# christian-rauch/MultiMotionFusion

Hardware: AMD Instinct MI355X
Metric: frames/sec @ 640x480 (dense ICP+RGB tracking + surfel fusion); Gauss-Newton iteration kernel (ICP + RGB JtJ-reduce) achieved HBM GB/s vs peak (higher is better)
Workload: dtype f32

## Files before the change

### include/mmf_hip.h

```cpp
#ifndef MMF_HIP_H_
#define MMF_HIP_H_

#include <stddef.h>
#include <stdint.h>

#ifdef __cplusplus
extern "C" {
#endif

#define MMF_ABI_VERSION 3

typedef enum {
    MMF_OK = 0,
    MMF_ERR_INVALID = -1,
    MMF_ERR_HIP = -2,
    MMF_ERR_NO_DEVICE = -3,
    MMF_ERR_STATE = -4
} mmf_status;

typedef struct mmf_ctx mmf_ctx;
typedef struct mmf_odom mmf_odom;

typedef struct {
    int16_t zero_x, zero_y;
// ... 248 lines not shown
int mmf_fusion_set_frame_to_frame_rgb(mmf_fusion *f, int val);
int mmf_fusion_set_depth_cutoff(mmf_fusion *f, float val);
int mmf_fusion_set_confidence_threshold(mmf_fusion *f, float val);
int mmf_fusion_set_enable_multiple_models(mmf_fusion *f, int val);
int mmf_fusion_get_config(mmf_fusion *f, mmf_fusion_config *out);
int mmf_fusion_set_shard(mmf_fusion *f, int rank, int world);
int mmf_fusion_owns_model(mmf_fusion *f, int index);
int mmf_fusion_set_model_pose(mmf_fusion *f, int index, const float pose[16]);
typedef struct mmf_shard mmf_shard;
int mmf_shard_unique_id(char id[128]);
int mmf_shard_create(mmf_ctx *ctx, int rank, int world, const char id[128], mmf_shard **out);
int mmf_shard_attach(mmf_ctx *ctx, int rank, int world, void *nccl_comm, mmf_shard **out);
void mmf_shard_destroy(mmf_shard *s);
int mmf_shard_broadcast_frame(mmf_shard *s, uint8_t *rgb, float *depth, uint8_t *mask, int width, int height, int root);
int mmf_shard_post_frame(mmf_shard *s, uint8_t *rgb, float *depth, uint8_t *mask, int width, int height, int root, int slot);
int mmf_shard_wait_frame(mmf_shard *s, int slot);
int mmf_shard_gather_poses(mmf_shard *s, mmf_fusion *f);
int mmf_shard_gather_poses_begin(mmf_shard *s, mmf_fusion *f);
int mmf_shard_gather_poses_end(mmf_shard *s, mmf_fusion *f);
int mmf_shard_gather_maps(mmf_shard *s, mmf_fusion *f, const int *labels, int spixel_size, float *out_dev);
int mmf_fusion_last_timings(mmf_fusion *f, double *tracking_s, double *frame_s);
int mmf_fusion_set_segmentation_callback(mmf_fusion *f, mmf_segmentation_fn fn, void *user);
int mmf_fusion_export_poses(mmf_fusion *f, const char *export_dir);
int mmf_fusion_pose_log(mmf_fusion *f, int index, long long *ts, float *p7, int max_entries, int *n_out);
int mmf_debug_expf(mmf_ctx *ctx, const float *x_dev, int n, float *out_mmf_dev, float *out_packed_dev);
int mmf_debug_set_gn_fused(int on);
int mmf_gn_chain_status(int *recoveries, int *one_launch_chain_in_use);
int mmf_debug_force_gn_fault(int n);
int mmf_debug_set_sparse_check(int on);
int mmf_debug_set_sparse_groups(int n);
int mmf_debug_odom_sparse_outside(mmf_odom *o, unsigned *outside, int *walked_by_extent, int rect[9]);
int mmf_debug_set_mid_predict(int on);
int mmf_debug_set_splat_bound(int mode);
int mmf_debug_set_pass_batch(int mode);
int mmf_debug_set_prep_rect(int on);
int mmf_debug_set_xcd(int on);
unsigned mmf_debug_xcd_block(unsigned block, unsigned blocks);
int mmf_debug_set_begin_rider(int on);
int mmf_debug_begin_rider_count(void);
int mmf_debug_set_track_cull(int mode);
int mmf_debug_depth_keys(mmf_ctx *ctx, const float *z_dev, int n, float max_depth, unsigned *fast_dev, unsigned *divided_dev);
int mmf_compute_fusion_weight(const float pose[16], const float last_pose[16], float multiplier, float *out);

int mmf_match_descriptors(mmf_ctx *ctx, const float *query, int nq, const float *train, int nt, int dim,
                          float max_distance, int *train_idx, float *distance);

typedef struct mmf_superpoint mmf_superpoint;
int mmf_superpoint_create(mmf_ctx *ctx, const float *const *weights, int max_width, int max_height,
                          int max_keypoints, mmf_superpoint **out);
void mmf_superpoint_destroy(mmf_superpoint *sp);
int mmf_superpoint_forward(mmf_superpoint *sp, const uint8_t *image, int width, int height, int channels);
int mmf_superpoint_download(mmf_superpoint *sp, int which, float *host, size_t count);
int mmf_superpoint_get_features(mmf_superpoint *sp, const uint8_t *image, int width, int height, int channels,
                                float conf_thresh, int nms_dist, int border, int *xy, float *conf, float *desc,
                                int *count);
int mmf_superpoint_conv(mmf_ctx *ctx, const float *in, int height, int width, int cin, const float *w,
                        const float *bias, int cout, int taps, int relu, int pool, int nt, float *out);

int mmf_slic_downsample(mmf_ctx *ctx, const int *labels, int width, int height, int spixel_size, const float *image,
                        int channels, int channel, int thresholded, float min_threshold, float *out, int *counts_out);
int mmf_slic_downsample_rgb(mmf_ctx *ctx, const int *labels, int width, int height, int spixel_size, const uint8_t *rgb,
                            int channels, uint8_t *out);
int mmf_slic_upsample_u8(mmf_ctx *ctx, const int *labels, int width, int height, const uint8_t *map, int nspix,
                         uint8_t *out);

typedef struct {
// ... 46 lines not shown
```

### multimotionfusion_amd/_capi.py

```python
import ctypes as C
import os

_PKG_DIR = os.path.dirname(os.path.abspath(__file__))
LIB_PATH = os.environ.get("MMF_HIP_LIB") or os.path.join(_PKG_DIR, "libmmf_hip.so")

MMF_NUM_PYRS = 3


class MmfError(RuntimeError):
    def __init__(self, status, message):
        super().__init__(f"mmf status {status}: {message}")
        self.status = status


class mmf_camera(C.Structure):
    _fields_ = [("fx", C.c_float), ("fy", C.c_float), ("cx", C.c_float), ("cy", C.c_float)]


class mmf_dataterm(C.Structure):
    _fields_ = [("zero_x", C.c_int16), ("zero_y", C.c_int16), ("one_x", C.c_int16), ("one_y", C.c_int16),
                ("diff", C.c_float), ("valid", C.c_uint8), ("pad_", C.c_uint8 * 3)]


class mmf_odom_stats(C.Structure):
# ... 176 lines not shown
                             _vp, C.POINTER(mmf_segmentation_model), _ip, _ip]),
    "mmf_crf_last": (_i, [_vp, C.POINTER(mmf_crf_info), C.POINTER(mmf_segmentation_model), _i, _vp, _vp, _vp, _vp]),
    "mmf_fusion_export_poses": (_i, [_vp, C.c_char_p]),
    "mmf_fusion_pose_log": (_i, [_vp, _i, C.POINTER(C.c_longlong), _fp, _i, _ip]),
    "mmf_compute_fusion_weight": (_i, [_fp, _fp, _f, _fp]),
    "mmf_fusion_preallocate_models": (_i, [_vp, C.c_uint]),
    "mmf_shard_unique_id": (_i, [C.c_char_p]),
    "mmf_shard_create": (_i, [_vp, _i, _i, C.c_char_p, C.POINTER(_vp)]),
    "mmf_shard_attach": (_i, [_vp, _i, _i, _vp, C.POINTER(_vp)]),
    "mmf_shard_destroy": (None, [_vp]),
    "mmf_shard_broadcast_frame": (_i, [_vp, _vp, _vp, _vp, _i, _i, _i]),
    "mmf_shard_post_frame": (_i, [_vp, _vp, _vp, _vp, _i, _i, _i, _i]),
    "mmf_shard_wait_frame": (_i, [_vp, _i]),
    "mmf_shard_gather_poses": (_i, [_vp, _vp]),
    "mmf_shard_gather_poses_begin": (_i, [_vp, _vp]),
    "mmf_shard_gather_poses_end": (_i, [_vp, _vp]),
    "mmf_shard_gather_maps": (_i, [_vp, _vp, _vp, _i, _vp]),
    "mmf_debug_expf": (_i, [_vp, _vp, _i, _vp, _vp]),
    "mmf_model_surfel_arrays": (_i, [_vp, C.POINTER(_vp), C.POINTER(_vp), C.POINTER(_vp), C.POINTER(C.c_uint)]),
    "mmf_debug_set_gn_fused": (_i, [_i]),
    "mmf_debug_set_mid_predict": (_i, [_i]),
    "mmf_debug_force_gn_fault": (_i, [_i]),
    "mmf_debug_set_sparse_check": (_i, [_i]),
    "mmf_debug_set_pass_batch": (_i, [_i]),
    "mmf_debug_set_prep_rect": (_i, [_i]),
    "mmf_debug_set_xcd": (_i, [_i]),
    "mmf_debug_xcd_block": (C.c_uint, [C.c_uint, C.c_uint]),
    "mmf_debug_set_begin_rider": (_i, [_i]),
    "mmf_debug_begin_rider_count": (_i, []),
    "mmf_debug_set_sparse_groups": (_i, [_i]),
    "mmf_debug_odom_sparse_outside": (_i, [_vp, C.POINTER(C.c_uint), C.POINTER(_i), C.POINTER(_i)]),
    "mmf_gn_chain_status": (_i, [C.POINTER(_i), C.POINTER(_i)]),
    "mmf_debug_set_splat_bound": (_i, [_i]),
    "mmf_debug_set_track_cull": (_i, [_i]),
    "mmf_debug_depth_keys": (_i, [_vp, _vp, _i, _f, _vp, _vp]),
    "mmf_fusion_set_shard": (_i, [_vp, _i, _i]),
    "mmf_fusion_owns_model": (_i, [_vp, _i]),
    "mmf_fusion_set_model_pose": (_i, [_vp, _i, _fp]),
    "mmf_fusion_last_timings": (_i, [_vp, C.POINTER(C.c_double), C.POINTER(C.c_double)]),
    "mmf_odom_enable_timing": (_i, [_vp, _i]),
    "mmf_odom_get_timing": (_i, [_vp, C.POINTER(mmf_odom_timing)]),
    "mmf_model_set_max_depth": (_i, [_vp, _f]),
    "mmf_model_set_confidence_threshold": (_i, [_vp, _f]),
    "mmf_model_confidence_threshold": (_f, [_vp]),
    "mmf_model_id": (_i, [_vp]),
}

_lib = None


def load():
    global _lib
    if _lib is not None:
        return _lib
    if not os.path.exists(LIB_PATH):
        raise ImportError(
            f"{LIB_PATH} is missing: build it with `python -m multimotionfusion_amd.build` "
            "(hipcc, gfx950). multimotionfusion_amd has no CPU fallback.")
    import torch
    lib = C.CDLL(LIB_PATH)
    for name, (restype, argtypes) in SIGNATURES.items():
        if os.environ.get("MMF_HIP_LIB") and name.startswith("mmf_debug_") and not hasattr(lib, name):
            continue
        fn = getattr(lib, name)
        fn.restype = restype
        fn.argtypes = argtypes
# ... 12 lines not shown
```

### multimotionfusion_amd/csrc/mmf_hip.hip

```cpp
#include "../../include/mmf_hip.h"

#include <hip/hip_runtime.h>
#include <hip/hip_ext.h>

#include <algorithm>
#include <array>
#include <atomic>
#include <cfloat>
#include <chrono>
#include <cmath>
#include <cstddef>
#include <cstdio>
#include <cstdlib>
#include <condition_variable>
#include <cstring>
#include <map>
#include <mutex>
#include <thread>
#include <new>
#include <string>
#include <tuple>
#include <type_traits>
#include <utility>
#include <vector>
// ... 2468 lines not shown
extern "C" int mmf_model_predict_indices(mmf_model* m, int time, float depth_cutoff, int time_delta) {
    return model_predict_indices(m, time, depth_cutoff, time_delta, false);
}

static unsigned* model_thumb_counts(mmf_model* m) { return &m->totals[4]; }
static dim3 splat_grid(size_t bound, bool deep = false) {
    const unsigned wgs = tunables().splat_wgs > 0 ? (unsigned)tunables().splat_wgs : (deep ? 2048u : 512u);
    const size_t one_per_thread = (bound + 255) / 256;
    return dim3((unsigned)std::max<size_t>(1, std::min<size_t>(one_per_thread, wgs)));
}
#ifdef MMF_SPLAT_COUNT
extern "C" int mmf_debug_splat_counts(unsigned long long out[4], int reset) {
    MMF_HIP_TRY(hipDeviceSynchronize());
    MMF_HIP_TRY(hipMemcpyFromSymbol(out, HIP_SYMBOL(g_splat_dbg), 32));
    if (reset) {
        const unsigned long long z[4] = {0, 0, 0, 0};
        MMF_HIP_TRY(hipMemcpyToSymbol(HIP_SYMBOL(g_splat_dbg), z, 32));
    }
    return MMF_OK;
}
#endif
extern "C" int mmf_debug_depth_keys(mmf_ctx* c, const float* z_dev, int n, float max_depth, unsigned* fast_dev, unsigned* divided_dev) {
    MMF_REQUIRE(c && z_dev && fast_dev && divided_dev && n > 0, "mmf_debug_depth_keys: bad argument");
    MMF_HIP_TRY(hipSetDevice(c->device));
    hipLaunchKernelGGL(depth_key_probe_kernel, grid1d((size_t)n), dim3(256), 0, c->stream, z_dev, n, max_depth, fast_dev, divided_dev);
    MMF_HIP_TRY(hipGetLastError());
    return MMF_OK;
}
static std::atomic<int> g_splat_bound{-2};
extern "C" int mmf_debug_set_splat_bound(int mode) {
    g_splat_bound.store(mode < 0 ? -1 : (mode ? 1 : 0));
    return MMF_OK;
}
static int model_combined_predict(mmf_model* m, float depth_cutoff, int time, int max_time, int time_delta,
                                  const uint8_t* fill_rgb, const float* fill_depth, int frame_to_frame_rgb, int lost) {
    MMF_REQUIRE(m != nullptr, "mmf_model_combined_predict: null model");
    mmf_ctx* c = m->ctx;
    MMF_HIP_TRY(hipSetDevice(c->device));
    ++m->tex_gen;
    ++m->thumb_gen;
    m->spl_nz_known = false;
    SplatArgs a;
    inverse4f_host(m->pose, a.t_inv.m);
    a.t_inv_dev = m->t_inv_dev;
    a.abort_dev = m->abort_dev;
    a.c = make_cam(m, false);
    a.cols = m->width, a.rows = m->height;
    a.maxDepth = depth_cutoff;
    a.confThreshold = m->conf_threshold;
    a.time = time, a.maxTime = max_time, a.timeDelta = time_delta;
    const unsigned launch_count = m->count_pending ? m->count_bound : m->count;
    const int bound_mode = g_splat_bound.load() == -2 ? tunables().splat_bound : g_splat_bound.load();
    const size_t npix_s = (size_t)m->width * m->height;
    const bool deep_store = (size_t)launch_count >= 2 * npix_s;
    const bool deep = bound_mode < 0 ? deep_store : bound_mode != 0;
    a.early_z = deep ? 1 : 0;
    a.rays = m->rays;
    const bool keep_box = m->boxes != nullptr && !(fill_rgb && fill_depth) && !deep && m->id != 0;
    if (keep_box) {
        ++m->kgen, ++m->sgen;
        const size_t plausible = std::min<size_t>(launch_count, (size_t)m->count * 2 + 8192);
        if (launch_count)
            hipLaunchKernelGGL(splat_box_kernel, splat_grid(plausible, plausible >= npix_s / 2), dim3(256), 0, c->stream, m->set[m->cur],
                               (int)launch_count, a, m->keys, m->count_pending ? m->totals : nullptr, m->boxes, m->kgen);
        hipLaunchKernelGGL(splat_resolve_keep_box_kernel, dim3(splat_tile_grid(m->width, m->height)), dim3(256), 0, c->stream, m->set[m->cur], a, m->keys,
                           m->image, m->vertexConf, m->normalRadius, m->time_tex, model_thumb_counts(m), (int)(m->thumb_gen & 1), m->boxes, m->kgen,
                           m->sgen);
        m->spl_nz_known = true;
        MMF_HIP_TRY(hipGetLastError());
        return MMF_OK;
    }
    if (launch_count)
        hipLaunchKernelGGL(deep ? splat_kernel<true> : splat_kernel<false>, splat_grid(launch_count, (size_t)launch_count >= npix_s / 2), dim3(256), 0, c->stream,
                           m->set[m->cur], (int)launch_count, a, m->keys, m->count_pending ? m->totals : nullptr);
    if (fill_rgb && fill_depth) {
        hipLaunchKernelGGL(splat_resolve_fill_kernel, dim3(splat_tile_grid(m->width, m->height)), dim3(256), 0,
                           c->stream, m->set[m->cur], a, m->keys, m->image, m->vertexConf, m->normalRadius, m->time_tex, fill_depth,
                           fill_rgb, lost ? 1 : 0, (lost || frame_to_frame_rgb) ? 1 : 0, m->fill_vertex, m->fill_normal,
                           m->fill_image, model_thumb_counts(m), (int)(m->thumb_gen & 1));
    } else
        hipLaunchKernelGGL(splat_resolve_kernel, dim3(splat_tile_grid(m->width, m->height)), dim3(256), 0, c->stream, m->set[m->cur], a, m->keys, m->image,
                           m->vertexConf, m->normalRadius, m->time_tex, model_thumb_counts(m), (int)(m->thumb_gen & 1));
    MMF_HIP_TRY(hipGetLastError());
    return MMF_OK;
}

extern "C" int mmf_model_combined_predict(mmf_model* m, float depth_cutoff, int time, int max_time, int time_delta) {
    return model_combined_predict(m, depth_cutoff, time, max_time, time_delta, nullptr, nullptr, 0, 0);
}

extern "C" int mmf_model_synthesize_depth(mmf_model* m, float depth_cutoff, float conf_threshold, int time, int max_time,
                                          int time_delta) {
    MMF_REQUIRE(m != nullptr, "mmf_model_synthesize_depth: null model");
    mmf_ctx* c = m->ctx;
    MMF_HIP_TRY(hipSetDevice(c->device));
    SplatArgs a;
    inverse4f_host(m->pose, a.t_inv.m);
    a.t_inv_dev = m->t_inv_dev;
    a.abort_dev = m->abort_dev;
    a.c = make_cam(m, false);
    a.cols = m->width, a.rows = m->height;
    a.maxDepth = depth_cutoff;
    a.confThreshold = conf_threshold;
    a.time = time, a.maxTime = max_time, a.timeDelta = time_delta;
    a.early_z = 0, a.rays = m->rays;
    if (int rc0 = model_resolve_count(m)) return rc0;
    if (m->count)
        hipLaunchKernelGGL(splat_kernel<false>, splat_grid(m->count), dim3(256), 0, c->stream, m->set[m->cur], (int)m->count, a,
                           m->keys, nullptr);
    hipLaunchKernelGGL(splat_depth_resolve_kernel, dim3(splat_tile_grid(m->width, m->height)), dim3(256), 0, c->stream, m->set[m->cur], a, m->keys,
                       m->synth_depth);
    MMF_HIP_TRY(hipGetLastError());
    return MMF_OK;
}

static int model_fuse(mmf_model* m, int time, const uint8_t* rgb, const uint8_t* mask, const float* depth_raw,
                      const float* depth_filtered, float depth_cutoff, float weighting, const IndexArgs* then_index) {
    MMF_REQUIRE(m && rgb && mask && depth_raw && depth_filtered, "mmf_model_fuse: null argument");
    if (int rc0 = model_resolve_count(m)) return rc0;
    mmf_ctx* c = m->ctx;
    MMF_HIP_TRY(hipSetDevice(c->device));
    FuseArgs a;
    std::memcpy(a.pose.m, m->pose, sizeof(m->pose));
    a.c = make_cam(m, true);
    a.cols = m->width, a.rows = m->height;
    a.time = time;
    a.weighting = weighting;
    a.pose_dev = m->pose_dev, a.weight_dev = m->weight_dev, a.weight_mult = weighting;
    a.abort_dev = m->abort_dev;
    a.maskID = m->id;
    a.maxDepth = depth_cutoff < m->max_depth ? depth_cutoff : m->max_depth;
    a.count = (int)m->count;
    hipLaunchKernelGGL(fuse_data_kernel, grid1d((size_t)((m->width + 1) / 2) * ((m->height + 1) / 2)), dim3(256), 0, c->stream, rgb, depth_raw, depth_filtered, mask,
                       m->index, m->vertConf, m->normRad, a, m->meas, m->flags_b, m->winner);
    if (m->count && then_index)
        hipLaunchKernelGGL(fuse_update_index_kernel, grid1d(m->count), dim3(256), 0, c->stream, m->set[m->cur], (int)m->count,
                           m->meas, time, m->winner, *then_index, m->keys);
    else if (m->count)
        hipLaunchKernelGGL(fuse_update_kernel, grid1d(m->count), dim3(256), 0, c->stream, m->set[m->cur], (int)m->count,
                           m->meas, time, m->winner);
    MMF_HIP_TRY(hipGetLastError());
// ... 127 lines not shown
    MMF_HIP_TRY(hipSetDevice(ms[0]->ctx->device));
    PassBatch<splat_box_item> b_splat;
    PassBatch<splat_resolve_rect_item> b_res;
    unsigned g_splat = 0;
    for (int k = 0; k < n; ++k) {
        mmf_model* m = ms[k];
        MMF_REQUIRE(m && m->boxes && m->rider.st == nullptr && !m->t_inv_dev && !m->abort_dev, "models_combined_predict_rect: a model with a device-side pose");
        ++m->tex_gen;
        ++m->thumb_gen;
        SplatArgs a;
        inverse4f_host(m->pose, a.t_inv.m);
        a.t_inv_dev = nullptr, a.abort_dev = nullptr;
        a.c = make_cam(m, false);
        a.cols = m->width, a.rows = m->height;
        a.maxDepth = depth_cutoff;
        a.confThreshold = m->conf_threshold;
        a.time = time, a.maxTime = max_time, a.timeDelta = time_delta;
        a.early_z = 0;
        a.rays = m->rays;
        const unsigned launch_count = m->count_pending ? m->count_bound : m->count;
        const size_t npix_s = (size_t)m->width * m->height;
        splat_box_item& sp = b_splat.m[k];
        sp.s = m->set[m->cur], sp.count = (int)launch_count, sp.a = a, sp.keys = m->keys, sp.count_dev = m->count_pending ? m->totals : nullptr;
        sp.boxes = m->boxes, sp.kgen = ++m->kgen;
        const size_t plausible = std::min<size_t>(launch_count, (size_t)m->count * 2 + 8192);
        sp.grid = launch_count ? splat_grid(plausible, plausible >= npix_s / 2).x : 0u;
        splat_resolve_rect_item& sr = b_res.m[k];
        sr.s = m->set[m->cur], sr.a = a, sr.keys = m->keys, sr.image = m->image, sr.vertexConf = m->vertexConf, sr.normalRadius = m->normalRadius,
        sr.time_out = m->time_tex, sr.thumb = model_thumb_counts(m), sr.gen = (int)(m->thumb_gen & 1);
        sr.boxes = m->boxes, sr.kgen = m->kgen, sr.sgen = ++m->sgen, sr.prev_whole = m->spl_nz_known ? 0 : 1;
        m->spl_nz_known = true;
        g_splat = std::max(g_splat, sp.grid);
    }
    if (g_splat) hipLaunchKernelGGL(splat_box_batched_kernel, dim3(g_splat, n), dim3(256), 0, st, b_splat);
    hipLaunchKernelGGL(splat_resolve_rect_batched_kernel, dim3(kRectGroups, n), dim3(256), 0, st, b_res);
    MMF_HIP_TRY(hipGetLastError());
    return MMF_OK;
}
static bool model_predict_batchable(const mmf_model* m) {
    const unsigned launch_count = m->count_pending ? m->count_bound : m->count;
    const int bound_mode = g_splat_bound.load() == -2 ? tunables().splat_bound : g_splat_bound.load();
    const bool deep = bound_mode < 0 ? (size_t)launch_count >= 2 * (size_t)m->width * m->height : bound_mode != 0;
    return !deep && m->rider.st == nullptr && !m->t_inv_dev && !m->abort_dev && !m->pose_dev;
}

extern "C" int mmf_model_perform_fill_in(mmf_model* m, const uint8_t* rgb, const float* depth_filtered,
                                         int frame_to_frame_rgb, int lost) {
    MMF_REQUIRE(m && rgb && depth_filtered, "mmf_model_perform_fill_in: null argument");
    ++m->tex_gen;
    mmf_ctx* c = m->ctx;
    MMF_HIP_TRY(hipSetDevice(c->device));
    const int npix = m->width * m->height;
    hipLaunchKernelGGL(fill_in_kernel, grid1d(npix), dim3(256), 0, c->stream, m->vertexConf, m->normalRadius, m->image,
                       depth_filtered, rgb, m->width, m->height, make_cam(m, false), lost ? 1 : 0,
                       (lost || frame_to_frame_rgb) ? 1 : 0, m->fill_vertex, m->fill_normal, m->fill_image);
    MMF_HIP_TRY(hipGetLastError());
    return MMF_OK;
}

extern "C" int mmf_model_requires_fill_in(mmf_model* m, float ratio, int* result) {
    MMF_REQUIRE(m && result, "mmf_model_requires_fill_in: null argument");
    mmf_ctx* c = m->ctx;
    MMF_HIP_TRY(hipSetDevice(c->device));
    const int dc = m->width / 20, dr = m->height / 20;
    MMF_HIP_TRY(hipMemsetAsync(&m->totals[2], 0, 4, c->stream));
    hipLaunchKernelGGL(thumbnail_count_kernel, grid1d(dc * dr), dim3(256), 0, c->stream, m->image, m->width, m->height,
                       &m->totals[2]);
// ... 538 lines not shown
```

### multimotionfusion_amd/csrc/pass_rect.hpp

```cpp
#pragma once
#include "extent.hpp"
#include "surfel_kernels.hpp"

namespace mmf {

constexpr int kRectGroups = 128;

constexpr int kMaxPassBatch = 7;
template <typename Item>
struct PassBatch {
    Item m[kMaxPassBatch];
};

__global__ __launch_bounds__(256) void mask_boxes_kernel(const uint8_t* __restrict__ mask, int cols, int rows, unsigned long long* __restrict__ boxes,
                                                         unsigned gen) {
    __shared__ int lo_x[256], hi_x[256], lo_y[256], hi_y[256];
    const int t = threadIdx.x;
    lo_x[t] = 0x7FFF, hi_x[t] = -1, lo_y[t] = 0x7FFF, hi_y[t] = -1;
    __syncthreads();
    const int tiles_x = (cols + 63) / 64;
    const int bx = blockIdx.x % tiles_x, by = blockIdx.x / tiles_x;
    const int x = bx * 64 + (t & 63);
#pragma unroll
    for (int r = 0; r < 4; ++r) {
// ... 210 lines not shown
        const unsigned k = base + (unsigned)__popcll(ballot & ((1ull << lane) - 1ull));
        if (k >= (unsigned)p.capacity) continue;
        const float2 ct = p.conf_time[c];
        if (old) {
            const float4 sp = p.s.pos[c], sc = p.s.col[c];
            p.dst.pos[k] = make_float4(sp.x, sp.y, sp.z, ct.x);
            p.dst.col[k] = make_float4(sc.x, sc.y, sc.z, ct.y);
            p.dst.nrm[k] = p.s.nrm[c];
        } else {
            const int d = clean_rect_candidate(c, count, mb, rows) - count;
            const float4 mp = p.meas.pos[d], mc = p.meas.col[d];
            p.dst.pos[k] = make_float4(mp.x, mp.y, mp.z, ct.x);
            p.dst.col[k] = make_float4(mc.x, mc.y, mc.z, ct.y);
            p.dst.nrm[k] = p.meas.nrm[d];
        }
    }
}

struct splat_box_item {
    SurfelSoA s;
    int count;
    SplatArgs a;
    unsigned long long* keys;
    const unsigned* count_dev;
    PassBoxes* boxes;
    unsigned kgen;
    unsigned grid;
};
__global__ __launch_bounds__(256) __attribute__((amdgpu_waves_per_eu(5))) void splat_box_batched_kernel(PassBatch<splat_box_item> b) {
    const splat_box_item& p = b.m[blockIdx.y];
    if (blockIdx.x >= p.grid) return;
    splat_kernel_body<false, true>(p.s, p.count, p.a, p.keys, p.count_dev, blockIdx.x, p.grid, p.boxes->key[p.kgen & 1u], p.kgen);
}

struct splat_resolve_rect_item {
    SurfelSoA s;
    SplatArgs a;
    unsigned long long* keys;
    uchar4* image;
    float4 *vertexConf, *normalRadius;
    unsigned short* time_out;
    unsigned* thumb;
    int gen;
    PassBoxes* boxes;
    unsigned kgen, sgen;
    int prev_whole;
};
__global__ __launch_bounds__(256) void splat_resolve_rect_batched_kernel(PassBatch<splat_resolve_rect_item> b) {
    const splat_resolve_rect_item& p = b.m[blockIdx.y];
    MMF_MODEL_STREAM_PRIORITY();
    const SplatArgs& a = p.a;
    const ExtentBox kb = box_clip(extent_load(p.boxes->key[p.kgen & 1u], p.kgen), a.cols, a.rows);
    const ExtentBox prev = p.prev_whole ? ExtentBox{0, 0, a.cols - 1, a.rows - 1} : box_of_ints(p.boxes->spl_nz[(p.sgen + 1u) & 1u]);
    const ExtentBox r = extent_hull(kb, prev);
    if (blockIdx.x == 0 && threadIdx.x == 0) {
        box_to_ints(p.boxes->spl_nz[p.sgen & 1u], kb);
        if (p.thumb) p.thumb[(p.gen + 1) & 1] = 0u;
    }
    if (r.x1 < r.x0 || r.y1 < r.y0) return;
    const int tiles_x = (a.cols + kSplatTile - 1) / kSplatTile;
    const int tx0 = r.x0 / kSplatTile, ty0 = r.y0 / kSplatTile, tw = r.x1 / kSplatTile - tx0 + 1, total = tw * (r.y1 / kSplatTile - ty0 + 1);
    for (int t = (int)blockIdx.x; t < total; t += (int)gridDim.x) {
        const int ty = t / tw;
        int px, py;
        unsigned long long k;
        const bool in = splat_tile_key(p.keys, a.cols, a.rows, px, py, k, 0u, (unsigned)((ty0 + ty) * tiles_x + tx0 + (t - ty * tw)));
// ... 14 lines not shown
```

### multimotionfusion_amd/csrc/surfel_kernels.hpp

```cpp
#pragma once
#include "extent.hpp"
#include <hip/hip_runtime.h>
#include <stdint.h>

#include "../../include/mmf_math.h"
#include "frame_rider.hpp"

#ifndef MMF_NO_PRIO
#define MMF_MODEL_STREAM_PRIORITY() __builtin_amdgcn_s_setprio(3)
#else
#define MMF_MODEL_STREAM_PRIORITY() do {} while (0)
#endif

namespace mmf {

struct v3 {
    float x, y, z;
};
__device__ __forceinline__ v3 V3(float x, float y, float z) { return v3{x, y, z}; }
__device__ __forceinline__ v3 v3add(v3 a, v3 b) { return V3(a.x + b.x, a.y + b.y, a.z + b.z); }
__device__ __forceinline__ v3 v3sub(v3 a, v3 b) { return V3(a.x - b.x, a.y - b.y, a.z - b.z); }
__device__ __forceinline__ v3 v3scale(v3 a, float s) { return V3(a.x * s, a.y * s, a.z * s); }
__device__ __forceinline__ float v3dot(v3 a, v3 b) { return a.x * b.x + a.y * b.y + a.z * b.z; }
__device__ __forceinline__ v3 v3cross(v3 a, v3 b) {
// ... 436 lines not shown
    if (i >= cols * rows) return;
    const int y = i / cols, x = i - y * cols;
    dst[i] = src[(size_t)x * rows + y];
}

#ifdef MMF_SPLAT_COUNT
__device__ unsigned long long g_splat_dbg[4];
#define MMF_SPLAT_TALLY(i, cond)                                                                                  \
    do {                                                                                                          \
        const unsigned long long b_ = __ballot(cond);                                                              \
        if (b_ && (threadIdx.x & 63u) == (unsigned)__builtin_ctzll(b_)) atomicAdd(&g_splat_dbg[i], (unsigned long long)__popcll(b_)); \
    } while (0)
#else
#define MMF_SPLAT_TALLY(i, cond) \
    do {                         \
    } while (0)
#endif
struct SplatArgs {
    Mat4 t_inv;
    const float* t_inv_dev;
    const int* abort_dev;
    Cam c;
    int cols, rows;
    float maxDepth, confThreshold;
    int time, maxTime, timeDelta;
    int early_z;
    const float4* rays;
};

struct SplatFrag {
    v3 h, nrm;
    float rad;
    int x0, x1, y0, y1;
    int cpx, cpy;
    unsigned dmin;
    float hn;
    bool ok;
};

template <bool SIZE = true>
__device__ __forceinline__ SplatFrag splat_setup(const float4 p, const float4 col, const float4 n, const SplatArgs& a, float* xw_out = nullptr,
                                                 float* yw_out = nullptr) {
    SplatFrag f;
    f.ok = false;
    f.h = m4point(a.t_inv, V3(p.x, p.y, p.z));
    const v3 h = f.h;
    if (h.z > a.maxDepth || h.z < 0 || p.w < a.confThreshold || (float)a.time - col.w > (float)a.timeDelta ||
        col.w > (float)a.maxTime)
        return f;
    const float fx = a.c.fx, fy = a.c.fy, cx = a.c.cx, cy = a.c.cy;
    const float xn = ((((fx * h.x) / h.z) + cx) - (a.cols * 0.5f)) / (a.cols * 0.5f);
    const float yn = ((((fy * h.y) / h.z) + cy) - (a.rows * 0.5f)) / (a.rows * 0.5f);
    const float zn = h.z / a.maxDepth;
    if (!(xn >= -1 && xn <= 1 && yn >= -1 && yn <= 1 && zn >= -1 && zn <= 1)) return f;
    f.nrm = v3normalize(m4dir(a.t_inv, V3(n.x, n.y, n.z)));
    f.rad = n.w;
    const v3 nrm = f.nrm;
    if (!SIZE) {
        f.hn = v3dot(h, nrm);
        f.x0 = f.y0 = 0, f.x1 = a.cols - 1, f.y1 = a.rows - 1, f.cpx = f.cpy = 0, f.dmin = 0u;
        if (xw_out) *xw_out = (xn + 1.0f) * (a.cols * 0.5f), *yw_out = (yn + 1.0f) * (a.rows * 0.5f);
        f.ok = true;
        return f;
    }
    const v3 x1 = v3scale(v3scale(v3normalize(V3((nrm.y - nrm.z), -nrm.x, nrm.x)), f.rad), 1.41421356f);
    const v3 y1 = v3cross(nrm, x1);
    const v3 q1 = v3add(h, x1), q2 = v3add(h, y1), q3 = v3sub(h, y1), q4 = v3sub(h, x1);
    const float p1x = ((fx * q1.x) / q1.z) + cx, p2x = ((fx * q2.x) / q2.z) + cx;
    const float p3x = ((fx * q3.x) / q3.z) + cx, p4x = ((fx * q4.x) / q4.z) + cx;
    const float p1y = ((fy * q1.y) / q1.z) + cy, p2y = ((fy * q2.y) / q2.z) + cy;
    const float p3y = ((fy * q3.y) / q3.z) + cy, p4y = ((fy * q4.y) / q4.z) + cy;
    const float xmin = fminf(p1x, fminf(p2x, fminf(p3x, p4x))), xmax = fmaxf(p1x, fmaxf(p2x, fmaxf(p3x, p4x)));
    const float ymin = fminf(p1y, fminf(p2y, fminf(p3y, p4y))), ymax = fmaxf(p1y, fmaxf(p2y, fmaxf(p3y, p4y)));
    float size = fmaxf(0.f, fmaxf(fabsf(xmax - xmin), fabsf(ymax - ymin)));
    if (!(size >= 1.0f)) size = 1.0f;
    const float xw = (xn + 1.0f) * (a.cols * 0.5f), yw = (yn + 1.0f) * (a.rows * 0.5f), hs = size * 0.5f;
    int x0 = (int)ceilf(xw - hs - 0.5f), x1i = (int)ceilf(xw + hs - 0.5f) - 1;
    int y0 = (int)ceilf(yw - hs - 0.5f), y1i = (int)ceilf(yw + hs - 0.5f) - 1;
    f.x0 = x0 < 0 ? 0 : x0, f.y0 = y0 < 0 ? 0 : y0;
    f.x1 = x1i > a.cols - 1 ? a.cols - 1 : x1i, f.y1 = y1i > a.rows - 1 ? a.rows - 1 : y1i;
    f.cpx = min(max((int)floorf(xw), f.x0), f.x1), f.cpy = min(max((int)floorf(yw), f.y0), f.y1);
    const float zlo = (h.z - f.rad) - (fabsf(h.z) + f.rad) * 4e-6f - 1e-7f;
    f.dmin = depth24((zlo / (2 * a.maxDepth)) + 0.5f);
    f.hn = v3dot(h, nrm);
    if (!(fabsf(f.hn) > 0.f)) f.dmin = 0u;
    f.ok = true;
    return f;
}

__device__ __forceinline__ v3 splat_ray(const Cam& c, int px, int py) {
    const float fcx = px + 0.5f, fcy = py + 0.5f;
    return v3normalize(V3((fcx - c.cx) / c.fx, (fcy - c.cy) / c.fy, 1.0f));
}
__device__ __forceinline__ float splat_plane_q(const SplatFrag& f, v3 l) { return f.hn / v3dot(l, f.nrm); }
__device__ __forceinline__ unsigned splat_depth24(float z, float maxDepth) { return depth24((z / (2 * maxDepth)) + 0.5f); }
__device__ __forceinline__ bool splat_in_disc(const SplatFrag& f, v3 l, float q) {
    const v3 diff = v3sub(v3scale(l, q), f.h);
    return !(v3dot(diff, diff) > f.rad * f.rad);
}
__device__ __forceinline__ bool splat_fragment(const SplatFrag& f, const SplatArgs& a, int px, int py, float& z,
                                               unsigned& d24) {
    const v3 l = splat_ray(a.c, px, py);
    const float q = splat_plane_q(f, l);
    if (!splat_in_disc(f, l, q)) return false;
    z = l.z * q;
    d24 = splat_depth24(z, a.maxDepth);
    return true;
}
__global__ __launch_bounds__(256) void splat_ray_kernel(Cam c, int cols, int rows, float4* __restrict__ rays) {
    const int i = blockIdx.x * 256 + threadIdx.x;
    if (i >= cols * rows) return;
    const int px = i / rows, py = i - px * rows;
    const v3 l = splat_ray(c, px, py);
    rays[i] = make_float4(l.x, l.y, l.z, 0.f);
}

struct SplatDepthScale {
// ... 17 lines not shown
}

constexpr int kSplatSeg = 4;
struct SplatRowLds {
    float nx[256], ny[256], nz[256], hn[256], hx[256], hy[256], hz[256], rad[256];
    unsigned x01[256];
    unsigned y0n[256];
    unsigned magic[256];
    unsigned dmin[256];
    int seg_end[256];
};
__device__ __forceinline__ int wave_min_all(int v) {
#pragma unroll
    for (int m = 1; m < 64; m <<= 1) v = min(v, __shfl_xor(v, m));
    return v;
}
__device__ __forceinline__ int wave_max_all(int v) {
#pragma unroll
    for (int m = 1; m < 64; m <<= 1) v = max(v, __shfl_xor(v, m));
    return v;
}
__device__ __forceinline__ void box_note_wave(unsigned long long* w, unsigned gen, bool valid, int x0, int x1, int y0, int y1) {
    const int a = wave_min_all(valid ? x0 : 0x7FFF), b = wave_max_all(valid ? x1 : -1);
    const int c = wave_min_all(valid ? y0 : 0x7FFF), d = wave_max_all(valid ? y1 : -1);
    if ((threadIdx.x & 63u) != 0u || b < a || d < c) return;
    const unsigned long long g = (unsigned long long)gen << 32;
    const unsigned long long v0 = g | (unsigned long long)(0xFFFF - a), v1 = g | (unsigned long long)b, v2 = g | (unsigned long long)(0xFFFF - c),
                             v3w = g | (unsigned long long)d;
    if (__hip_atomic_load(&w[0], __ATOMIC_RELAXED, __HIP_MEMORY_SCOPE_AGENT) < v0) atomicMax(&w[0], v0);
    if (__hip_atomic_load(&w[1], __ATOMIC_RELAXED, __HIP_MEMORY_SCOPE_AGENT) < v1) atomicMax(&w[1], v1);
    if (__hip_atomic_load(&w[2], __ATOMIC_RELAXED, __HIP_MEMORY_SCOPE_AGENT) < v2) atomicMax(&w[2], v2);
    if (__hip_atomic_load(&w[3], __ATOMIC_RELAXED, __HIP_MEMORY_SCOPE_AGENT) < v3w) atomicMax(&w[3], v3w);
}
template <bool EARLYZ, bool BOX = false>
__device__ __forceinline__ void splat_kernel_body(SurfelSoA s, int count, SplatArgs a_in,
                                                    unsigned long long* __restrict__ keys,
                                                    const unsigned* __restrict__ count_dev, const unsigned bx_, [[maybe_unused]] const unsigned gx_,
                                                    [[maybe_unused]] unsigned long long* key_box = nullptr, [[maybe_unused]] unsigned kgen = 0u) {
    MMF_MODEL_STREAM_PRIORITY();
    MMF_SPECULATION_GUARD(a_in);
    int bx0 = 0x7FFF, bx1 = -1, by0 = 0x7FFF, by1 = -1;
    const SplatArgs a = with_device_pose(a_in);
    __shared__ SplatRowLds L;
    const int lane = threadIdx.x & 63, wbase = threadIdx.x & ~63;
    if (count_dev != nullptr) count = min((unsigned)count, *count_dev);
    const int nwaves = (int)gx_ * 4, wave_id = (int)bx_ * 4 + (int)(threadIdx.x >> 6);
    const int per = min(64, max(1, (count + nwaves - 1) / nwaves));
    const SplatDepthScale ds = splat_depth_scale(a.maxDepth);
    for (int base = wave_id * per; base < count; base += nwaves * per) {
        const int id = base + lane;
        SplatFrag f;
        f.ok = false;
        if (lane < per && id < count) {
            const float4 p = s.pos[id], col = s.col[id], n = s.nrm[id];
            asm volatile("" ::"v"(col.w), "v"(n.w));
            f = splat_setup(p, col, n, a);
        }
        const int h = f.ok ? max(f.y1 - f.y0 + 1, 0) : 0, w = f.ok ? max(f.x1 - f.x0 + 1, 0) : 0;
        if (BOX && h > 0 && w > 0) bx0 = min(bx0, f.x0), bx1 = max(bx1, f.x1), by0 = min(by0, f.y0), by1 = max(by1, f.y1);
        const int nseg = (w + kSplatSeg - 1) / kSplatSeg;
        int scan = h * nseg;
#pragma unroll
        for (int d = 1; d < 64; d <<= 1) {
            const int up = __shfl_up(scan, d);
            if (lane >= d) scan += up;
        }
        const int total = __shfl(scan, 63);
        if (total == 0) continue;
        asm volatile("s_waitcnt lgkmcnt(0)" ::: "memory");
        __builtin_amdgcn_wave_barrier();
        {
            const int t = threadIdx.x;
            L.nx[t] = f.nrm.x, L.ny[t] = f.nrm.y, L.nz[t] = f.nrm.z, L.hn[t] = f.hn;
            L.hx[t] = f.h.x, L.hy[t] = f.h.y, L.hz[t] = f.h.z, L.rad[t] = f.rad;
            L.x01[t] = (unsigned)f.x0 | ((unsigned)f.x1 << 16);
            L.y0n[t] = (unsigned)f.y0 | ((unsigned)nseg << 16);
            L.magic[t] = nseg > 1 ? 0xFFFFFFFFu / (unsigned)nseg + 1u : 0u;
            if (EARLYZ) L.dmin[t] = f.dmin;
            L.seg_end[t] = scan;
        }
        asm volatile("s_waitcnt lgkmcnt(0)" ::: "memory");
        __builtin_amdgcn_wave_barrier();
        for (int t = lane; t < total; t += 64) {
            int lo = 0, hi = 63;
#pragma unroll
            for (int step = 0; step < 6; ++step) {
                const int mid = (lo + hi) >> 1;
                const bool right = L.seg_end[wbase + mid] <= t;
                lo = right ? mid + 1 : lo;
                hi = right ? hi : mid;
            }
            const int e = wbase + lo;
            const unsigned local = (unsigned)(t - (lo ? L.seg_end[e - 1] : 0));
            const unsigned x01 = L.x01[e], y0n = L.y0n[e], magic = L.magic[e];
            const unsigned row = magic ? __umulhi(local, magic) : local;
            const unsigned sx = local - row * (y0n >> 16);
            const int py = (int)(y0n & 0xFFFFu) + (int)row, pb = (int)(x01 & 0xFFFFu) + kSplatSeg * (int)sx, x1 = (int)(x01 >> 16);
            const unsigned sid = (unsigned)(base + lo);
            SplatFrag g;
            g.nrm = V3(L.nx[e], L.ny[e], L.nz[e]), g.hn = L.hn[e];
            g.h = V3(L.hx[e], L.hy[e], L.hz[e]), g.rad = L.rad[e];
            const unsigned dmin = EARLYZ ? L.dmin[e] : 0u;

            unsigned zbv[kSplatSeg];
            float4 ray[kSplatSeg];
#pragma unroll
            for (int k = 0; k < kSplatSeg; ++k) {
                const size_t at = (size_t)min(pb + k, x1) * a.rows + py;
                zbv[k] = EARLYZ ? (unsigned)(__hip_atomic_load(&keys[at], __ATOMIC_RELAXED, __HIP_MEMORY_SCOPE_AGENT) >> 32) : 0xFFFFFFFFu;
                ray[k] = a.rays[at];
            }
            unsigned d24v[kSplatSeg];
            bool draw[kSplatSeg];
#pragma unroll
            for (int k = 0; k < kSplatSeg; ++k) {
                const v3 l = V3(ray[k].x, ray[k].y, ray[k].z);
                const float q = splat_plane_q(g, l);
                d24v[k] = splat_depth24_fast(l.z * q, ds);
                draw[k] = pb + k <= x1 && !(EARLYZ && (dmin > zbv[k] || d24v[k] > zbv[k])) && splat_in_disc(g, l, q);
                MMF_SPLAT_TALLY(0, pb + k <= x1);
                MMF_SPLAT_TALLY(2, draw[k]);
            }
#pragma unroll
            for (int k = 0; k < kSplatSeg; ++k)
                if (draw[k]) atomicMin(&keys[(size_t)(pb + k) * a.rows + py], ((unsigned long long)d24v[k] << 32) | sid);
        }
    }
    if (BOX) box_note_wave(key_box, kgen, bx1 >= bx0 && by1 >= by0, bx0, bx1, by0, by1);
}
__global__ __launch_bounds__(256) __attribute__((amdgpu_waves_per_eu(5))) void splat_box_kernel(SurfelSoA s, int count, SplatArgs a_in,
                                                    unsigned long long* __restrict__ keys, const unsigned* __restrict__ count_dev,
                                                    PassBoxes* boxes, unsigned kgen) {
    splat_kernel_body<false, true>(s, count, a_in, keys, count_dev, blockIdx.x, gridDim.x, boxes->key[kgen & 1u], kgen);
}
template <bool EARLYZ>
__global__ __launch_bounds__(256) __attribute__((amdgpu_waves_per_eu(5))) void splat_kernel(SurfelSoA s, int count, SplatArgs a_in,
                                                    unsigned long long* __restrict__ keys,
                                                    const unsigned* __restrict__ count_dev) {
    splat_kernel_body<EARLYZ>(s, count, a_in, keys, count_dev, blockIdx.x, gridDim.x);
}


struct SplatTexel {
    uchar4 image;
    float4 vertexConf, normalRadius;
    unsigned short time;
};

constexpr int kSplatTile = 16;
__device__ __forceinline__ bool splat_tile_key(unsigned long long* __restrict__ keys, int cols, int rows, int& px, int& py,
                                               unsigned long long& k, unsigned first_block = 0, unsigned block = ~0u) {
    __shared__ unsigned long long tile[kSplatTile][kSplatTile + 1];
    const int tiles_x = (cols + kSplatTile - 1) / kSplatTile;
    const int bid = (int)((block == ~0u ? blockIdx.x : block) - first_block);
    const int bx = bid % tiles_x, by = bid / tiles_x;
    const int t = threadIdx.x;
    {
        const int cx = t >> 4, cy = t & 15;
        const int x = bx * kSplatTile + cx, y = by * kSplatTile + cy;
        unsigned long long v = kEmptyKey;
        if (x < cols && y < rows) {
            v = keys[(size_t)x * rows + y];
            if (v != kEmptyKey) keys[(size_t)x * rows + y] = kEmptyKey;
        }
        tile[cx][cy] = v;
    }
    __syncthreads();
    const int ly = t >> 4, lx = t & 15;
    px = bx * kSplatTile + lx, py = by * kSplatTile + ly;
    k = tile[lx][ly];
    return px < cols && py < rows;
}
// ... 695 lines not shown
```

Measured before the change: 2925.

## Tighten splat screen bounds to the projected disc ellipse extent

Computes an analytic bounding box of each surfel's projected disc per axis and clamps the square splat footprint to it, so fewer pixels are visited and tested per surfel during splatting. It falls back to the old square box when the conic is degenerate. A debug check mode counts covered pixels that fall outside the tight box, to validate conservativeness. It also raises the waves-per-EU hint for the non-early-Z splat kernel. The extra per-surfel setup math and possible missed edge pixels are the tradeoffs.

```diff
diff --git a/include/mmf_hip.h b/include/mmf_hip.h
--- a/include/mmf_hip.h
+++ b/include/mmf_hip.h
@@ -304,6 +304,8 @@
 int mmf_debug_odom_sparse_outside(mmf_odom *o, unsigned *outside, int *walked_by_extent, int rect[9]);
 int mmf_debug_set_mid_predict(int on);
 int mmf_debug_set_splat_bound(int mode);
+int mmf_debug_set_splat_check(int on);
+int mmf_debug_get_splat_outside(mmf_ctx *ctx, unsigned long long counts[5], int reset);
 int mmf_debug_set_pass_batch(int mode);
 int mmf_debug_set_prep_rect(int on);
 int mmf_debug_set_xcd(int on);
diff --git a/multimotionfusion_amd/_capi.py b/multimotionfusion_amd/_capi.py
--- a/multimotionfusion_amd/_capi.py
+++ b/multimotionfusion_amd/_capi.py
@@ -232,6 +232,8 @@
     "mmf_debug_odom_sparse_outside": (_i, [_vp, C.POINTER(C.c_uint), C.POINTER(_i), C.POINTER(_i)]),
     "mmf_gn_chain_status": (_i, [C.POINTER(_i), C.POINTER(_i)]),
     "mmf_debug_set_splat_bound": (_i, [_i]),
+    "mmf_debug_set_splat_check": (_i, [_i]),
+    "mmf_debug_get_splat_outside": (_i, [_vp, C.POINTER(C.c_ulonglong), _i]),
     "mmf_debug_set_track_cull": (_i, [_i]),
     "mmf_debug_depth_keys": (_i, [_vp, _vp, _i, _f, _vp, _vp]),
     "mmf_fusion_set_shard": (_i, [_vp, _i, _i]),
diff --git a/multimotionfusion_amd/csrc/mmf_hip.hip b/multimotionfusion_amd/csrc/mmf_hip.hip
--- a/multimotionfusion_amd/csrc/mmf_hip.hip
+++ b/multimotionfusion_amd/csrc/mmf_hip.hip
@@ -2524,6 +2524,22 @@
     g_splat_bound.store(mode < 0 ? -1 : (mode ? 1 : 0));
     return MMF_OK;
 }
+static std::atomic<int> g_splat_check_on{0};
+extern "C" int mmf_debug_set_splat_check(int on) {
+    g_splat_check_on.store(on ? 1 : 0);
+    return MMF_OK;
+}
+extern "C" int mmf_debug_get_splat_outside(mmf_ctx* c, unsigned long long counts[5], int reset) {
+    MMF_REQUIRE(c && counts, "mmf_debug_get_splat_outside: null argument");
+    MMF_HIP_TRY(hipSetDevice(c->device));
+    MMF_HIP_TRY(hipDeviceSynchronize());
+    MMF_HIP_TRY(hipMemcpyFromSymbol(counts, HIP_SYMBOL(g_splat_check), 40));
+    if (reset) {
+        const unsigned long long z[5] = {0, 0, 0, 0, 0};
+        MMF_HIP_TRY(hipMemcpyToSymbol(HIP_SYMBOL(g_splat_check), z, 40));
+    }
+    return MMF_OK;
+}
 static int model_combined_predict(mmf_model* m, float depth_cutoff, int time, int max_time, int time_delta,
                                   const uint8_t* fill_rgb, const float* fill_depth, int frame_to_frame_rgb, int lost) {
     MMF_REQUIRE(m != nullptr, "mmf_model_combined_predict: null model");
@@ -2549,11 +2565,12 @@
     a.early_z = deep ? 1 : 0;
     a.rays = m->rays;
     const bool keep_box = m->boxes != nullptr && !(fill_rgb && fill_depth) && !deep && m->id != 0;
+    const bool check = g_splat_check_on.load() != 0;
     if (keep_box) {
         ++m->kgen, ++m->sgen;
         const size_t plausible = std::min<size_t>(launch_count, (size_t)m->count * 2 + 8192);
         if (launch_count)
-            hipLaunchKernelGGL(splat_box_kernel, splat_grid(plausible, plausible >= npix_s / 2), dim3(256), 0, c->stream, m->set[m->cur],
+            hipLaunchKernelGGL(check ? splat_box_check_kernel : splat_box_kernel, splat_grid(plausible, plausible >= npix_s / 2), dim3(256), 0, c->stream, m->set[m->cur],
                                (int)launch_count, a, m->keys, m->count_pending ? m->totals : nullptr, m->boxes, m->kgen);
         hipLaunchKernelGGL(splat_resolve_keep_box_kernel, dim3(splat_tile_grid(m->width, m->height)), dim3(256), 0, c->stream, m->set[m->cur], a, m->keys,
                            m->image, m->vertexConf, m->normalRadius, m->time_tex, model_thumb_counts(m), (int)(m->thumb_gen & 1), m->boxes, m->kgen,
@@ -2563,7 +2580,7 @@
         return MMF_OK;
     }
     if (launch_count)
-        hipLaunchKernelGGL(deep ? splat_kernel<true> : splat_kernel<false>, splat_grid(launch_count, (size_t)launch_count >= npix_s / 2), dim3(256), 0, c->stream,
+        hipLaunchKernelGGL(check ? (deep ? splat_check_kernel<true> : splat_check_kernel<false>) : (deep ? splat_kernel<true> : splat_kernel<false>), splat_grid(launch_count, (size_t)launch_count >= npix_s / 2), dim3(256), 0, c->stream,
                            m->set[m->cur], (int)launch_count, a, m->keys, m->count_pending ? m->totals : nullptr);
     if (fill_rgb && fill_depth) {
         hipLaunchKernelGGL(splat_resolve_fill_kernel, dim3(splat_tile_grid(m->width, m->height)), dim3(256), 0,
@@ -2598,7 +2615,7 @@
     a.early_z = 0, a.rays = m->rays;
     if (int rc0 = model_resolve_count(m)) return rc0;
     if (m->count)
-        hipLaunchKernelGGL(splat_kernel<false>, splat_grid(m->count), dim3(256), 0, c->stream, m->set[m->cur], (int)m->count, a,
+        hipLaunchKernelGGL(g_splat_check_on.load() ? splat_check_kernel<false> : splat_kernel<false>, splat_grid(m->count), dim3(256), 0, c->stream, m->set[m->cur], (int)m->count, a,
                            m->keys, nullptr);
     hipLaunchKernelGGL(splat_depth_resolve_kernel, dim3(splat_tile_grid(m->width, m->height)), dim3(256), 0, c->stream, m->set[m->cur], a, m->keys,
                        m->synth_depth);
@@ -2792,7 +2809,7 @@
         m->spl_nz_known = true;
         g_splat = std::max(g_splat, sp.grid);
     }
-    if (g_splat) hipLaunchKernelGGL(splat_box_batched_kernel, dim3(g_splat, n), dim3(256), 0, st, b_splat);
+    if (g_splat) hipLaunchKernelGGL(g_splat_check_on.load() ? splat_box_batched_check_kernel : splat_box_batched_kernel, dim3(g_splat, n), dim3(256), 0, st, b_splat);
     hipLaunchKernelGGL(splat_resolve_rect_batched_kernel, dim3(kRectGroups, n), dim3(256), 0, st, b_res);
     MMF_HIP_TRY(hipGetLastError());
     return MMF_OK;
diff --git a/multimotionfusion_amd/csrc/pass_rect.hpp b/multimotionfusion_amd/csrc/pass_rect.hpp
--- a/multimotionfusion_amd/csrc/pass_rect.hpp
+++ b/multimotionfusion_amd/csrc/pass_rect.hpp
@@ -266,6 +266,11 @@
     if (blockIdx.x >= p.grid) return;
     splat_kernel_body<false, true>(p.s, p.count, p.a, p.keys, p.count_dev, blockIdx.x, p.grid, p.boxes->key[p.kgen & 1u], p.kgen);
 }
+__global__ __launch_bounds__(256) void splat_box_batched_check_kernel(PassBatch<splat_box_item> b) {
+    const splat_box_item& p = b.m[blockIdx.y];
+    if (blockIdx.x >= p.grid) return;
+    splat_kernel_body<false, true, true>(p.s, p.count, p.a, p.keys, p.count_dev, blockIdx.x, p.grid, p.boxes->key[p.kgen & 1u], p.kgen);
+}
 
 struct splat_resolve_rect_item {
     SurfelSoA s;
diff --git a/multimotionfusion_amd/csrc/surfel_kernels.hpp b/multimotionfusion_amd/csrc/surfel_kernels.hpp
--- a/multimotionfusion_amd/csrc/surfel_kernels.hpp
+++ b/multimotionfusion_amd/csrc/surfel_kernels.hpp
@@ -492,13 +492,53 @@
     v3 h, nrm;
     float rad;
     int x0, x1, y0, y1;
+    int rx0, rx1, ry0, ry1;
+    bool fallback;
     int cpx, cpy;
     unsigned dmin;
     float hn;
     bool ok;
 };
 
-template <bool SIZE = true>
+struct SplatAxis {
+    float lo, hi;
+    bool ok;
+};
+__device__ __forceinline__ SplatAxis splat_disc_axis(float c0, float nc, float no, float nz, float rho2, float A, float iA, float f, float c) {
+    const float m = nc - c0 * nz;
+    const float k1 = c0 * no, k2 = c0 * nc + nz;
+    const float K = (k1 * k1 + k2 * k2) + no * no;
+    const float B = rho2 * (c0 + m * nz);
+    const float D = B * B + A * (rho2 * K);
+    const float sq = sqrtf(D);
+    const float lo = f * (c0 + (B - sq) * iA) + c, hi = f * (c0 + (B + sq) * iA) + c;
+    const float mg = 2e-3f + 1e-5f * (fabsf(lo - c) + fabsf(hi - c));
+    SplatAxis r;
+    r.lo = ceilf((lo - mg) - 0.5f), r.hi = floorf((hi + mg) - 0.5f);
+    r.ok = D > 0.f && fabsf(r.lo) <= 3e38f && fabsf(r.hi) <= 3e38f;
+    return r;
+}
+__device__ __forceinline__ void splat_disc_box(SplatFrag& f, const SplatArgs& a, float hs) {
+    const v3 h = f.h, n = f.nrm;
+    f.rx0 = f.x0, f.rx1 = f.x1, f.ry0 = f.y0, f.ry1 = f.y1;
+    f.fallback = true;
+    const float ahn = fabsf(f.hn), rad = fabsf(f.rad), h2 = v3dot(h, h);
+    const float R = rad + (4e-6f * (h2 + rad * rad)) / ahn;
+    const float tx = hs * a.c.ifx, ty = hs * a.c.ify;
+    const float s2 = h2 * (tx * tx + ty * ty);
+    if (!(ahn > 0.f && ahn <= 3e38f && R < 0.9f * h.z && ahn * ahn > 4.0f * s2)) return;
+    const float ihz = 1.0f / h.z, rho = R * ihz, rho2 = rho * rho;
+    const float A = (1.0f - rho2) + rho2 * (n.z * n.z), iA = 1.0f / A;
+    const SplatAxis X = splat_disc_axis(h.x * ihz, n.x, n.y, n.z, rho2, A, iA, a.c.fx, a.c.cx);
+    if (!X.ok) return;
+    const SplatAxis Y = splat_disc_axis(h.y * ihz, n.y, n.x, n.z, rho2, A, iA, a.c.fy, a.c.cy);
+    if (!Y.ok) return;
+    f.fallback = false;
+    f.x0 = (int)fminf(fmaxf(X.lo, (float)f.rx0), (float)(f.rx1 + 1)), f.x1 = (int)fmaxf(fminf(X.hi, (float)f.rx1), (float)(f.x0 - 1));
+    f.y0 = (int)fminf(fmaxf(Y.lo, (float)f.ry0), (float)(f.ry1 + 1)), f.y1 = (int)fmaxf(fminf(Y.hi, (float)f.ry1), (float)(f.y0 - 1));
+}
+
+template <bool SIZE = true, bool TIGHT = true>
 __device__ __forceinline__ SplatFrag splat_setup(const float4 p, const float4 col, const float4 n, const SplatArgs& a, float* xw_out = nullptr,
                                                  float* yw_out = nullptr) {
     SplatFrag f;
@@ -539,10 +579,16 @@
     int y0 = (int)ceilf(yw - hs - 0.5f), y1i = (int)ceilf(yw + hs - 0.5f) - 1;
     f.x0 = x0 < 0 ? 0 : x0, f.y0 = y0 < 0 ? 0 : y0;
     f.x1 = x1i > a.cols - 1 ? a.cols - 1 : x1i, f.y1 = y1i > a.rows - 1 ? a.rows - 1 : y1i;
+    f.hn = v3dot(h, nrm);
+    splat_disc_box(f, a, hs);
+    if (!TIGHT) {
+        const int tx0 = f.x0, tx1 = f.x1, ty0 = f.y0, ty1 = f.y1;
+        f.x0 = f.rx0, f.x1 = f.rx1, f.y0 = f.ry0, f.y1 = f.ry1;
+        f.rx0 = tx0, f.rx1 = tx1, f.ry0 = ty0, f.ry1 = ty1;
+    }
     f.cpx = min(max((int)floorf(xw), f.x0), f.x1), f.cpy = min(max((int)floorf(yw), f.y0), f.y1);
     const float zlo = (h.z - f.rad) - (fabsf(h.z) + f.rad) * 4e-6f - 1e-7f;
     f.dmin = depth24((zlo / (2 * a.maxDepth)) + 0.5f);
-    f.hn = v3dot(h, nrm);
     if (!(fabsf(f.hn) > 0.f)) f.dmin = 0u;
     f.ok = true;
     return f;
@@ -626,7 +672,11 @@
     if (__hip_atomic_load(&w[2], __ATOMIC_RELAXED, __HIP_MEMORY_SCOPE_AGENT) < v2) atomicMax(&w[2], v2);
     if (__hip_atomic_load(&w[3], __ATOMIC_RELAXED, __HIP_MEMORY_SCOPE_AGENT) < v3w) atomicMax(&w[3], v3w);
 }
-template <bool EARLYZ, bool BOX = false>
+__device__ unsigned long long g_splat_check[5];
+__device__ __forceinline__ void splat_check_add(int i, bool cond, unsigned n = 1u) {
+    if (cond) atomicAdd(&g_splat_check[i], (unsigned long long)n);
+}
+template <bool EARLYZ, bool BOX = false, bool CHECK = false>
 __device__ __forceinline__ void splat_kernel_body(SurfelSoA s, int count, SplatArgs a_in,
                                                     unsigned long long* __restrict__ keys,
                                                     const unsigned* __restrict__ count_dev, const unsigned bx_, [[maybe_unused]] const unsigned gx_,
@@ -636,6 +686,7 @@
     int bx0 = 0x7FFF, bx1 = -1, by0 = 0x7FFF, by1 = -1;
     const SplatArgs a = with_device_pose(a_in);
     __shared__ SplatRowLds L;
+    __shared__ unsigned tight_x01[CHECK ? 256 : 1], tight_y01[CHECK ? 256 : 1];
     const int lane = threadIdx.x & 63, wbase = threadIdx.x & ~63;
     if (count_dev != nullptr) count = min((unsigned)count, *count_dev);
     const int nwaves = (int)gx_ * 4, wave_id = (int)bx_ * 4 + (int)(threadIdx.x >> 6);
@@ -648,7 +699,12 @@
         if (lane < per && id < count) {
             const float4 p = s.pos[id], col = s.col[id], n = s.nrm[id];
             asm volatile("" ::"v"(col.w), "v"(n.w));
-            f = splat_setup(p, col, n, a);
+            f = splat_setup<true, !CHECK>(p, col, n, a);
+        }
+        if (CHECK && f.ok) {
+            splat_check_add(1, f.fallback), splat_check_add(2, true);
+            splat_check_add(3, true, (unsigned)(max(f.x1 - f.x0 + 1, 0) * max(f.y1 - f.y0 + 1, 0)));
+            splat_check_add(4, true, (unsigned)(max(f.rx1 - f.rx0 + 1, 0) * max(f.ry1 - f.ry0 + 1, 0)));
         }
         const int h = f.ok ? max(f.y1 - f.y0 + 1, 0) : 0, w = f.ok ? max(f.x1 - f.x0 + 1, 0) : 0;
         if (BOX && h > 0 && w > 0) bx0 = min(bx0, f.x0), bx1 = max(bx1, f.x1), by0 = min(by0, f.y0), by1 = max(by1, f.y1);
@@ -671,6 +727,10 @@
             L.y0n[t] = (unsigned)f.y0 | ((unsigned)nseg << 16);
             L.magic[t] = nseg > 1 ? 0xFFFFFFFFu / (unsigned)nseg + 1u : 0u;
             if (EARLYZ) L.dmin[t] = f.dmin;
+            if (CHECK) {
+                tight_x01[t] = (unsigned)f.rx0 | ((unsigned)(f.rx1 + 1) << 16);
+                tight_y01[t] = (unsigned)f.ry0 | ((unsigned)(f.ry1 + 1) << 16);
+            }
             L.seg_end[t] = scan;
         }
         asm volatile("s_waitcnt lgkmcnt(0)" ::: "memory");
@@ -712,7 +772,14 @@
                 const float q = splat_plane_q(g, l);
                 d24v[k] = splat_depth24_fast(l.z * q, ds);
                 draw[k] = pb + k <= x1 && !(EARLYZ && (dmin > zbv[k] || d24v[k] > zbv[k])) && splat_in_disc(g, l, q);
+                if (CHECK) {
+                    const unsigned tx = tight_x01[e], ty = tight_y01[e];
+                    const bool in_box = pb + k >= (int)(tx & 0xFFFFu) && pb + k < (int)(tx >> 16) && py >= (int)(ty & 0xFFFFu) && py < (int)(ty >> 16);
+                    splat_check_add(0, pb + k <= x1 && !in_box && splat_in_disc(g, l, q));
+                }
                 MMF_SPLAT_TALLY(0, pb + k <= x1);
+                MMF_SPLAT_TALLY(1, pb + k <= x1 && !(EARLYZ && dmin > zbv[k]));
+                MMF_SPLAT_TALLY(3, true);
                 MMF_SPLAT_TALLY(2, draw[k]);
             }
 #pragma unroll
@@ -728,10 +795,19 @@
     splat_kernel_body<false, true>(s, count, a_in, keys, count_dev, blockIdx.x, gridDim.x, boxes->key[kgen & 1u], kgen);
 }
 template <bool EARLYZ>
-__global__ __launch_bounds__(256) __attribute__((amdgpu_waves_per_eu(5))) void splat_kernel(SurfelSoA s, int count, SplatArgs a_in,
+__global__ __launch_bounds__(256) __attribute__((amdgpu_waves_per_eu(EARLYZ ? 5 : 6))) void splat_kernel(SurfelSoA s, int count, SplatArgs a_in,
                                                     unsigned long long* __restrict__ keys,
                                                     const unsigned* __restrict__ count_dev) {
     splat_kernel_body<EARLYZ>(s, count, a_in, keys, count_dev, blockIdx.x, gridDim.x);
+}
+template <bool EARLYZ>
+__global__ __launch_bounds__(256) void splat_check_kernel(SurfelSoA s, int count, SplatArgs a_in, unsigned long long* __restrict__ keys,
+                                                          const unsigned* __restrict__ count_dev) {
+    splat_kernel_body<EARLYZ, false, true>(s, count, a_in, keys, count_dev, blockIdx.x, gridDim.x);
+}
+__global__ __launch_bounds__(256) void splat_box_check_kernel(SurfelSoA s, int count, SplatArgs a_in, unsigned long long* __restrict__ keys,
+                                                              const unsigned* __restrict__ count_dev, PassBoxes* boxes, unsigned kgen) {
+    splat_kernel_body<false, true, true>(s, count, a_in, keys, count_dev, blockIdx.x, gridDim.x, boxes->key[kgen & 1u], kgen);
 }
 
 
```

New measurement: 2915, median of 2. Within noise of the previous version (-0.3%).
